# jeong0982/gkr

Measured on AMD Instinct MI355X. Metric: BN254-Fr sumcheck field-ops/sec @ 2^20 vars, higher is better.
Workload: dtype u32x8

## Files before the change

gkr_amd/csrc/capi_internal.h:

```cpp
#pragma once
#include <hip/hip_runtime.h>
#include <sched.h>
#include <stdio.h>
#include <stdlib.h>
#include <string.h>

#include <algorithm>
#include <chrono>
#include <condition_variable>
#include <map>
#include <memory>
#include <mutex>
#include <string>
#include <thread>
#include <vector>

#include "../../include/gkr_amd.h"
#include "fr64.h"
#include "host_cpus.h"
#include "hostpool.h"
#include "kernels.h"
#include "options.h"
#include "gate_seg.h"
#include "keccak.h"
// ... 151 lines not shown
        for (auto p : r) (void)hipFree(p);
        for (auto& g : lists) g.release();
        gt.clear();
        l.clear();
        r.clear();
        lists.clear();
    }
};

struct ProveCrew;

struct AsyncWorker {
    std::thread th;
    std::mutex mu;
    std::condition_variable cv;
    std::function<void()> task;
    bool busy = false, stop = false;
    void loop() {
        std::unique_lock<std::mutex> g(mu);
        for (;;) {
            cv.wait(g, [this] { return stop || (busy && task); });
            if (stop) return;
            std::function<void()> t = std::move(task);
            task = nullptr;
            g.unlock();
            t();
            g.lock();
            busy = false;
            cv.notify_all();
        }
    }
    void run(std::function<void()> fn) {
        std::unique_lock<std::mutex> g(mu);
        if (!th.joinable()) th = std::thread([this] { loop(); });
        cv.wait(g, [this] { return !busy; });
        task = std::move(fn);
        busy = true;
        cv.notify_all();
    }
    void wait() {
        std::unique_lock<std::mutex> g(mu);
        cv.wait(g, [this] { return !busy; });
    }
    ~AsyncWorker() {
        {
            std::unique_lock<std::mutex> g(mu);
            cv.wait(g, [this] { return !busy; });
            stop = true;
            cv.notify_all();
        }
        if (th.joinable()) th.join();
    }
};

struct gkr_ctx {
    int device = 0;
    std::vector<int> devices;
    int host_threads = 0;
    gkr::Options options = gkr::Options::from_environment();
    std::vector<std::unique_ptr<PreparedCircuit>> circuits;
    hipStream_t stream = nullptr;
    hipStream_t aux = nullptr;
    hipStream_t late = nullptr;
    hipStream_t chain = nullptr;
    std::vector<hipEvent_t> aux_events;
    Fr* d_cts = nullptr;
    int transcript = GKR_TRANSCRIPT_HOST;
    std::string err;
    int profile = 0;
    std::map<std::string, ProfileRow> prof;
    std::vector<PendingEvent> pending;
    std::vector<hipEvent_t> event_pool;
    char name[256] = {0};
    uint32_t ticket = 0;
    std::unique_ptr<gkr::SpinPool> pool;
    std::unique_ptr<gkr::SpinPool> solo_pool;
    std::unique_ptr<AsyncWorker> copier;
    std::unique_ptr<AsyncWorker> liner;
    void* mle_arrivals_zeroed = nullptr;
    void* arrivals_zeroed = nullptr;
    void* gate_arrive_zeroed = nullptr;
    bool crew_member = false;
    int help_share = 0;
    int rounds_ahead = 0;
    std::unique_ptr<ProveCrew, void (*)(ProveCrew*)> crew{nullptr, nullptr};
    std::map<std::string, std::pair<void*, size_t>> ws;
    std::map<std::string, std::pair<void*, size_t>> pinned;

    hipError_t workspace(const char* slot, size_t bytes, void** out) {
        auto& e = ws[slot];
        if (e.second < bytes) {
            if (e.first) (void)device_free(e.first);
            e.first = nullptr;
            e.second = 0;
            hipError_t rc = device_malloc(&e.first, bytes);
            if (rc != hipSuccess) return rc;
            e.second = bytes;
        }
        *out = e.first;
        return hipSuccess;
    }
    hipError_t pinned_host(const char* slot, size_t bytes, void** out) {
        auto& e = pinned[slot];
        if (e.second < bytes) {
            if (e.first) (void)hipHostFree(e.first);
            e.first = nullptr;
            e.second = 0;
            hipError_t rc = hipHostMalloc(&e.first, bytes, hipHostMallocCoherent | hipHostMallocMapped);
            if (rc != hipSuccess) return rc;
            memset(e.first, 0, bytes);
            e.second = bytes;
        }
        *out = e.first;
        return hipSuccess;
    }
    void release_buffers() {
        for (auto& c : circuits) c->release();
        circuits.clear();
        for (auto& kv : ws)
            if (kv.second.first) (void)device_free(kv.second.first);
        ws.clear();
        for (auto& kv : pinned)
            if (kv.second.first) (void)hipHostFree(kv.second.first);
        pinned.clear();
    }
    int threads() const { return host_threads > 0 ? host_threads : default_host_threads(); }
    gkr::SpinPool* host_pool() {
        if (crew_member) {
            if (!solo_pool) solo_pool.reset(new gkr::SpinPool(0));
            return solo_pool.get();
        }
        if (!pool) pool.reset(new gkr::SpinPool(threads() - 1));
        return pool.get();
    }
    hipError_t late_stream(hipStream_t* out) {
        if (!late) {
            const hipError_t rc = hipStreamCreateWithFlags(&late, hipStreamNonBlocking);
            if (rc != hipSuccess) return rc;
        }
        *out = late;
        return hipSuccess;
    }
    hipError_t chain_stream(hipStream_t* out) {
        if (!chain) {
            hipError_t rc = hipStreamCreateWithFlags(&chain, hipStreamNonBlocking);
            if (rc != hipSuccess) return rc;
        }
        *out = chain;
        return hipSuccess;
    }
    hipError_t aux_stream(int events) {
        if (!aux) {
            hipError_t rc = hipStreamCreateWithFlags(&aux, hipStreamNonBlocking);
            if (rc != hipSuccess) return rc;
        }
        while ((int)aux_events.size() < events) {
            hipEvent_t e;
            hipError_t rc = hipEventCreateWithFlags(&e, hipEventDisableTiming);
            if (rc != hipSuccess) return rc;
            aux_events.push_back(e);
        }
        return hipSuccess;
    }

    int fail(int status, const std::string& what) {
        err = what;
// ... 77 lines not shown
        }
    }
};

#define GKR_ENTER(ctx)                                        \
    HIP_TRY(ctx, hipSetDevice((ctx)->device));                \
    gkr::OptionScope gkr_option_scope_(&(ctx)->options)

#define HIP_TRY(ctx, expr)                                   \
    do {                                                     \
        hipError_t _e = (expr);                              \
        if (_e != hipSuccess) return (ctx)->hip_fail(_e, #expr); \
    } while (0)


namespace gkr_host {


template <typename T>
struct DevBuf {
    T* p = nullptr;
    ~DevBuf() {
        if (p) (void)hipFree(p);
    }
    hipError_t alloc(size_t count) { return hipMalloc(reinterpret_cast<void**>(&p), count * sizeof(T)); }
};

template <typename Run>
int run_on_upload(gkr_ctx* ctx, const gkr_fr* host, size_t count, Run run) {
    GKR_ENTER(ctx);
    DevBuf<Fr> d;
    HIP_TRY(ctx, d.alloc(count));
    HIP_TRY(ctx, hipMemcpyAsync(d.p, host, count * sizeof(Fr), hipMemcpyHostToDevice, ctx->stream));
    return run(d.p);
}
template <typename Run>
int run_on_tables(gkr_ctx* ctx, const gkr_fr* tables, size_t count, Run run) {
    if (!all_canonical(tables, count)) return ctx->fail(GKR_ERR_NON_CANONICAL, "table entry >= r");
    return run_on_upload(ctx, tables, count, run);
}

struct ThreadTimeAccount {
    double own_pieces_us = 0, helped_us = 0, spin_us = 0;
};
inline thread_local ThreadTimeAccount t_account;
struct HostAccountTotals {
    std::atomic<uint64_t> own_ns{0}, helped_ns{0}, spin_ns{0}, rest_ns{0}, lent_ns{0}, lent_idle_ns{0}, calls{0}, wake_ns{0};
    std::atomic<uint64_t> pieces{0}, piece_ns{0}, piece_pass_ns{0}, lanes[17] = {};
    std::atomic<bool> on{false};
};
inline HostAccountTotals& host_account_totals() {
    static HostAccountTotals t;
    return t;
}
inline bool accounting_on() { return host_account_totals().on.load(std::memory_order_relaxed); }
inline void account_piece(int transcripts, double pass_us, double total_us) {
    HostAccountTotals& t = host_account_totals();
    t.pieces.fetch_add(1, std::memory_order_relaxed);
    t.piece_ns.fetch_add((uint64_t)(total_us * 1e3), std::memory_order_relaxed);
    t.piece_pass_ns.fetch_add((uint64_t)(pass_us * 1e3), std::memory_order_relaxed);
    t.lanes[transcripts < 1 ? 1 : (transcripts > 16 ? 16 : transcripts)].fetch_add(1, std::memory_order_relaxed);
}
inline double now_us_dbg() { return std::chrono::duration<double, std::micro>(std::chrono::steady_clock::now().time_since_epoch()).count(); }

inline bool help_enabled() {
    static const bool on = !gkr::process_switch("GKR_NO_HELP");
    return on;
}
static void run_pieces(gkr::SpinPool* pool, const std::function<bool()>* work, bool several, int priority = 0) {
    auto run = [&] {
        if (pool)
            pool->run_now(work);
        else
            while ((*work)()) {
            }
    };
    const bool dbg = gkr::debug_timing() || accounting_on();
    const double t0 = dbg ? now_us_dbg() : 0.0;
    if (several && help_enabled()) {
        gkr::HelpBoard::Posted posted(work, priority);
        run();
    } else {
        run();
    }
    if (dbg) t_account.own_pieces_us += now_us_dbg() - t0;
}

template <typename Rec>
inline int wait_records(gkr_ctx* ctx, const volatile Rec* recs, int count, uint32_t ticket) {
    const auto t0 = std::chrono::steady_clock::now();
    const bool help = help_enabled();
    auto last_progress = t0;
    for (int b = 0; b < count; ++b) {
        uint32_t spins = 0, helped = 0;
        while (__atomic_load_n(&recs[b].seq, __ATOMIC_ACQUIRE) != ticket) {
            const bool dbg = gkr::debug_timing() || accounting_on();
            const double th0 = dbg ? now_us_dbg() : 0.0;
            const bool did_help = help && gkr::HelpBoard::instance().help();
            if (!did_help) GKR_CPU_RELAX();
            if (dbg) (did_help ? t_account.helped_us : t_account.spin_us) += now_us_dbg() - th0;
            if (did_help ? (++helped & 0x3F) == 0 : (++spins & 0xFFFF) == 0) {
                hipError_t q = hipStreamQuery(ctx->stream);
                if (q != hipSuccess && q != hipErrorNotReady) return ctx->hip_fail(q, "stream failed while waiting for a round");
                if (std::chrono::steady_clock::now() - last_progress > std::chrono::seconds(30)) {
                    if (q == hipSuccess && __atomic_load_n(&recs[b].seq, __ATOMIC_ACQUIRE) == ticket) break;
                    return ctx->fail(GKR_ERR_HIP, "timed out waiting for the device to publish a round");
                }
            }
        }
        if (spins | helped) last_progress = std::chrono::steady_clock::now();
    }
    return GKR_OK;
}

constexpr int kMaxGroups = 32;
constexpr int kMleShardTailLog2 = 6;

#define WS(ctx, slot, type, count, ptr) \
    HIP_TRY(ctx, (ctx)->workspace(slot, (size_t)(count) * sizeof(type), reinterpret_cast<void**>(&(ptr))))

inline int mle_pass_rounds(int m, int n, int jmax) {
    int j = m < jmax ? m : jmax;
    if (((size_t)1 << m) > gkr::kSmallPassEntries && m != n && j > m - 6) j = m - 6;
    if (jmax > 3 && (m - j == 10 || m - j == 11) && m - 12 >= 1) j = m - 12;
    return j < 1 ? 1 : j;
}

constexpr int kMleFirstFoldLevels = 2;
constexpr int kMleTwoLevelRounds = 2 * gkr::kMlePassMaxRounds;
inline bool mle_two_level_first_fold(int n, const gkr::Options& o) {
    const long long levels = o.v[gkr::OPT_first_fold_levels] == 1 || o.v[gkr::OPT_first_fold_levels] == 2 ? o.v[gkr::OPT_first_fold_levels] : kMleFirstFoldLevels;
    return levels == 2 && n >= 18 && n <= 24 && !o.v[gkr::OPT_no_mfma_fold] && o.v[gkr::OPT_rounds_per_pass] <= 0;
}

inline void write_round_output(gkr_fr* out_coeffs, uint32_t* out_len, gkr_fr* out_r, size_t row, const void* c0, const void* c1, uint32_t ln,
                               const void* r) {
    memset(&out_coeffs[row * 2], 0, 32);
    if (ln == 2) memcpy(&out_coeffs[row * 2], c1, 32);
    memcpy(&out_coeffs[row * 2 + 1], c0, 32);
    out_len[row] = ln;
    memcpy(&out_r[row], r, 32);
}
struct GroupHandoff {
    int b0 = 0, nb = 0;
    int state = 0;
    uint32_t ticket = 0;
    std::atomic<uint64_t> claim{0};
    std::atomic<int> done{0};
    template <typename Rec>
    bool records_landed(const Rec* rec) const {
        for (int i = nb - 1; i >= 0; --i)
            if (__atomic_load_n(&rec[b0 + i].seq, __ATOMIC_ACQUIRE) != ticket) return false;
        return true;
    }
    void open(uint32_t generation) {
        done.store(0, std::memory_order_relaxed);
        claim.store((uint64_t)generation << 32, std::memory_order_release);
        state = 1;
    }
    uint32_t open_generation() const {
        const uint64_t c = claim.load(std::memory_order_acquire);
        return (uint32_t)c < (uint32_t)nb ? (uint32_t)(c >> 32) : 0u;
    }
    bool try_claim(uint32_t chunk, uint32_t* first, uint32_t* take, uint32_t* generation = nullptr) {
        uint64_t c = claim.load(std::memory_order_acquire);
        while ((c >> 32) != 0 && (uint32_t)c < (uint32_t)nb) {
// ... 124 lines not shown
```

gkr_amd/csrc/capi_layer.hip:

```cpp
#include "capi_internal.h"

namespace gkr_host {

void host_prod_pass_scalar(const uint64_t* recs, size_t rec_row_words, int count, int J, const uint32_t (*vec_len)[16],
                                  uint64_t (*c2)[16][4], uint64_t (*lin)[16][4], uint64_t (*c0)[16][4], uint64_t (*r)[16][4],
                                  uint64_t* weights, size_t w_row_words) {
    using namespace gkr::h64;
    const F* cts = host_mimc_constants64();
    const F one_m = to_mont(F{{1, 0, 0, 0}});
    for (int k = 0; k < count; ++k) {
        F M[64], SY[8], rm[gkr::kProdMaxJ];
        const F* rec = reinterpret_cast<const F*>(recs + (size_t)k * rec_row_words);
        const int n = 1 << J;
        for (int a = 0; a < n; ++a) {
            for (int b = 0; b < n; ++b) M[a * 8 + b] = rec[a * 8 + b];
            SY[a] = rec[64 + a];
        }
        for (int t = 0; t < J; ++t) {
            const int half = 1 << (J - t - 1);
            F p00 = M[0], p01 = M[half], p10 = M[half * 8], p11 = M[half * 8 + half], s0 = SY[0], s1 = SY[half];
            for (int x = 1; x < half; ++x) {
                p00 = add(p00, M[x * 8 + x]);
                p01 = add(p01, M[x * 8 + half + x]);
                p10 = add(p10, M[(half + x) * 8 + x]);
// ... 201 lines not shown
    return GKR_OK;
}

struct RankExchange {
    gkr_ctx* ctx;
    const LayerShardArgs* shard;
    hipStream_t s;
    uint32_t* h_xflag = nullptr;
    int sums = 0;

    int sum(Fr* d_a, Fr* d_b, size_t each, const uint32_t* d_flag, int local_fail) {
        ++sums;
        if (shard->dev) {
            Timed t(ctx, "exchange", 0.0);
            long long* limbs = reinterpret_cast<long long*>(shard->dev->d_limbs);
            gkr::launch_exchange_widen(d_a, d_b, (uint32_t)each, d_flag, local_fail ? 1u : 0u, limbs, s);
            const int arc = shard->dev->fn(shard->dev->user, (2 * each + 1) * 8, static_cast<void*>(s));
            gkr::launch_exchange_narrow(limbs, d_a, d_b, (uint32_t)each, h_xflag, s);
            if (arc) return ctx->fail(GKR_ERR_INVALID, "the device sum-over-ranks hook failed (status " + std::to_string(arc) + ")");
            HIP_TRY(ctx, hipGetLastError());
            return local_fail;
        }
        const auto t0 = std::chrono::steady_clock::now();
        gkr_fr* buf = nullptr;
        HIP_TRY(ctx, ctx->pinned_host("layer.xbuf", sizeof(gkr_fr) * (2 * each + 1), reinterpret_cast<void**>(&buf)));
        uint32_t hflag = local_fail ? 1u : 0u;
        gkr::launch_copy_words(d_a, buf, each * 8, s);
        gkr::launch_copy_words(d_b, buf + each, each * 8, s);
        if (d_flag && !local_fail && hipMemcpyAsync(&hflag, d_flag, 4, hipMemcpyDeviceToHost, s) != hipSuccess) hflag = 1u;
        const hipError_t se = hipStreamSynchronize(s);
        if (se != hipSuccess) hflag = 1u;
        buf[2 * each] = gkr_fr{{(uint64_t)(hflag != 0), 0, 0, 0}};
        const int arc = shard->allreduce(shard->user, buf, 2 * each + 1);
        if (se != hipSuccess) return ctx->hip_fail(se, "hipStreamSynchronize before the sum over ranks");
        if (arc) return ctx->fail(GKR_ERR_INVALID, "the sum-over-ranks hook failed (status " + std::to_string(arc) + ")");
        if (!all_canonical(buf, 2 * each + 1)) return ctx->fail(GKR_ERR_NON_CANONICAL, "the sum-over-ranks hook returned a value >= r");
        const bool some_failed = (buf[2 * each].l[0] | buf[2 * each].l[1] | buf[2 * each].l[2] | buf[2 * each].l[3]) != 0;
        gkr::launch_copy_words(buf, d_a, each * 8, s);
        gkr::launch_copy_words(buf + each, d_b, each * 8, s);
        if (ctx->profile == 1)
            ctx->add_host_sample("exchange", std::chrono::duration<double, std::milli>(std::chrono::steady_clock::now() - t0).count());
        if (local_fail) return local_fail;
        if (some_failed) return ctx->fail(GKR_ERR_INVALID, "gate type or operand index out of range, or another failure, on some rank");
        return GKR_OK;
    }
    bool flagged() const { return h_xflag && __atomic_load_n(h_xflag, __ATOMIC_ACQUIRE); }
    int check() const { return flagged() ? ctx->fail(GKR_ERR_INVALID, "gate type or operand index out of range, or another failure, on some rank") : GKR_OK; }
};

static int queue_c_phase_setup(LayerRun& R, const LayerPinned& P, RankExchange& xch, uint32_t jp, bool wu_in_host_tail, gkr_fr* const* out_r) {
    const uint32_t k = (uint32_t)R.k, k_i = (uint32_t)R.k_i, batch = (uint32_t)R.batch;
    for (uint32_t b = 0; b < batch; ++b) memcpy(P.u + (size_t)b * k, out_r[b], sizeof(gkr_fr) * k);
    const gkr::CPhaseFuse fuse{wu_in_host_tail ? P.tail : R.Wb, P.pw, R.X, R.Y, jp};
    gkr::launch_eq_table(reinterpret_cast<const Fr*>(P.u), k, 0u, k, R.eq, true, batch, R.s, R.wu ? &fuse : nullptr, R.wu,
                         (uint32_t)(wu_in_host_tail ? 3 * P.tail_stride() : R.wlen));
    bool c_tables_done = false;
    {
        Timed t(R.ctx, "gate_rows", (double)R.span.count * 8.0 * batch);
        if (R.wide) {
            const gkr::WideCFuse wfuse{R.wu, R.X, R.Y};
            gkr::launch_gate_rows_wide(R.span, k_i, k, R.g->plan, R.gate_eq(), R.eq, R.A, R.M, R.lb, R.item_partials, R.gate_arrive, R.s, R.sets, R.plan_counts,
                                       R.wu ? &wfuse : nullptr);
            c_tables_done = R.wu != nullptr;
        } else
            c_tables_done = gkr::launch_gate_rows(R.span, k_i, k, R.g->offsets, R.g->cursor, R.g->list, R.e_hi, R.e_lo, R.kl, R.eq, R.A, R.M, R.lb, &R.g->segs,
                                                  R.seg_partials, R.s, R.shard ? nullptr : &fuse, R.sets);
    }
    if (R.shard)
        if (const int rc = xch.sum(R.A, R.M, R.wlen, nullptr, GKR_OK)) return rc;
    if (!c_tables_done) gkr::launch_prod_c_setup(R.Wb, jp, P.pw, R.A, R.M, R.X, R.Y, k, (uint32_t)R.wlen, batch, R.s);
    return GKR_OK;
}

struct HostPass {
    const LayerPinned* pin;
    int batch, k;
    bool ifma;
    gkr_fr* const* out_coeffs;
    uint32_t* const* out_len;
    gkr_fr* const* out_r;
    uint32_t J, round0, tail_m, tail_jp;
    bool on_host;
    int chunk;
    std::atomic<int> next{0};
};

static bool host_pass_piece(HostPass& hp) {
    const LayerPinned& P = *hp.pin;
    const int first = hp.next.fetch_add(hp.chunk, std::memory_order_relaxed);
    if (first >= hp.batch) return false;
    const int cnt = hp.batch - first < hp.chunk ? hp.batch - first : hp.chunk;
    uint64_t c2[gkr::kProdMaxJ][16][4], lin[gkr::kProdMaxJ][16][4], c0[gkr::kProdMaxJ][16][4], rr[gkr::kProdMaxJ][16][4];
    uint32_t vl[gkr::kProdMaxJ][16];
    const bool acct = accounting_on();
    const double tp0 = acct ? now_us_dbg() : 0.0;
    if (hp.on_host)
        for (int i = 0; i < cnt; ++i)
            host_tail_pass(reinterpret_cast<gkr::h64::F*>(P.tail + (size_t)(first + i) * 3 * P.tail_stride()), P.tail_stride(), hp.tail_m, hp.tail_jp,
                           reinterpret_cast<const gkr::h64::F*>(P.pw + (size_t)(first + i) * 8), hp.J, reinterpret_cast<gkr::h64::F*>(&P.prec[first + i].v[0]));
    for (uint32_t t = 0; t < hp.J; ++t)
        for (int i = 0; i < cnt; ++i) vl[t][i] = 2u + (P.dep[(size_t)(first + i) * 32 + (hp.round0 + t) % hp.k] ? 1u : 0u);
    (hp.ifma && cnt >= 3 ? gkr::gkr_ifma_prod_pass : host_prod_pass_scalar)(
        reinterpret_cast<const uint64_t*>(P.prec + first), sizeof(gkr::ProdPassRec) / 8, cnt, (int)hp.J, vl, c2, lin, c0, rr,
        reinterpret_cast<uint64_t*>(P.pw + (size_t)first * 8), 32);
    const double tp1 = acct ? now_us_dbg() : 0.0;
    for (int i = 0; i < cnt; ++i) {
        const int b = first + i;
        for (uint32_t t = 0; t < hp.J; ++t) {
            const uint32_t round = hp.round0 + t;
            gkr_fr* oc = hp.out_coeffs[b] + (size_t)round * 3;
            memset(&oc[0], 0, 32);
            if (vl[t][i] == 3) memcpy(&oc[0], c2[t][i], 32);
            memcpy(&oc[1], lin[t][i], 32);
            memcpy(&oc[2], c0[t][i], 32);
            hp.out_len[b][round] = vl[t][i];
            memcpy(&hp.out_r[b][round], rr[t][i], 32);
        }
    }
    if (acct) account_piece(cnt, tp1 - tp0, now_us_dbg() - tp0);
    return true;
}

static int run_layer_passes(LayerRun& R, const LayerPinned& P, RankExchange& xch, gkr_fr* const* out_coeffs, uint32_t* const* out_len, gkr_fr* const* out_r) {
    gkr_ctx* ctx = R.ctx;
    const int batch = R.batch, k = R.k;
    Fr* d_ppart = nullptr;
    WS(ctx, "layer.ppart", Fr, (size_t)batch * gkr::prod_pass_scratch_values((uint32_t)k), d_ppart);
    unsigned char* d_fold_plans = nullptr;
    if (k >= 14) WS(ctx, "layer.foldplans", unsigned char, (size_t)batch * gkr::prod_fold_plan_bytes(), d_fold_plans);
    uint32_t* d_arrivals = nullptr;
    if (!gkr::opt(gkr::OPT_no_fused_publish)) {
        WS(ctx, "layer.arrivals", uint32_t, (size_t)(batch < 4096 ? 4096 : batch), d_arrivals);
        if (ctx->arrivals_zeroed != d_arrivals) {
            HIP_TRY(ctx, hipMemsetAsync(d_arrivals, 0, sizeof(uint32_t) * (size_t)(batch < 4096 ? 4096 : batch), R.s));
            ctx->arrivals_zeroed = d_arrivals;
        }
    }
    gkr::SpinPool* pool = batch >= 16 ? ctx->host_pool() : nullptr;
    const bool ifma = host_ifma_ready();
    const bool dbg_sections = gkr::debug_timing();
    double us_launch = 0, us_wait = 0, us_pieces = 0, us_phase1 = 0;
    const double t_passes0 = dbg_sections ? now_us_dbg() : 0.0;
    gkr::SpinPool::Session session(pool, nullptr);
    uint32_t round0 = 0, jp = 0, tail_m = 0;
    bool tail_active = false;
    int rc = GKR_OK;
    for (int phase = 0; phase < 2 && rc == GKR_OK; ++phase) {
        if (phase == 1) {
            const bool wu_in_host_tail = tail_active && R.wu;
            if (tail_active && !wu_in_host_tail) gkr::launch_copy_rows(P.tail, 3 * P.tail_stride() * 8, R.Wb, R.wlen * 8, 8u << jp, (uint32_t)batch, R.s);
            const double t_ph1 = dbg_sections ? now_us_dbg() : 0.0;
            rc = queue_c_phase_setup(R, P, xch, jp, wu_in_host_tail, out_r);
            if (dbg_sections) us_phase1 += now_us_dbg() - t_ph1;
            if (rc) break;
            jp = 0;
            tail_active = false;
        }
        Fr *const Tw = phase ? R.Wc : R.Wb, *const Tx = phase ? R.X : R.U, *const Ty = phase ? R.Y : R.V;
        uint32_t m = (uint32_t)k;
        for (uint32_t rem = (uint32_t)k; rem > 0 && rc == GKR_OK;) {
            const uint32_t J = rem < (uint32_t)gkr::kProdMaxJ ? rem : (uint32_t)gkr::kProdMaxJ;
            const bool on_host = tail_active;
            const bool exports = P.tail && !on_host && m - jp <= P.tail_log2 && rem > J;
            if (!on_host) {
                const uint32_t ticket = ++ctx->ticket;
                const double tl0 = dbg_sections ? now_us_dbg() : 0.0;
                {
                    Timed t(ctx, "layer_prod_pass", 0.0);
                    gkr::launch_prod_pass(Tw, Tx, Ty, m, jp, P.pw, J, d_ppart, (uint32_t)R.wlen, P.prec, ticket, (uint32_t)batch, R.s, d_arrivals, d_fold_plans,
                                          exports ? P.tail : nullptr, (uint32_t)P.tail_stride());
                }
                if (hipError_t le = hipGetLastError(); le != hipSuccess) {
                    rc = ctx->hip_fail(le, "launch of a layer pass");
                    break;
                }
                const double tl1 = dbg_sections ? now_us_dbg() : 0.0;
                rc = wait_records(ctx, P.prec, batch, ticket);
                if (dbg_sections) {
                    us_launch += tl1 - tl0;
                    us_wait += now_us_dbg() - tl1;
                }
                if (!rc) rc = xch.check();
                if (rc) break;
            }
            const int chunk = hash_chunk_size(batch, pool ? pool->workers() + 1 : 1, ctx->crew_member ? ctx->help_share : 0);
            HostPass hp{&P, batch, k, ifma, out_coeffs, out_len, out_r, J, round0, on_host ? tail_m : 0u, jp, on_host, chunk};
            const std::function<bool()> work = [&hp]() -> bool { return host_pass_piece(hp); };
            m -= jp;
            const double tw0 = dbg_sections ? now_us_dbg() : 0.0;
            run_pieces(pool, &work, batch > chunk, ctx->rounds_ahead + (int)(2 * k - round0));
            if (dbg_sections) us_pieces += now_us_dbg() - tw0;
            if (exports) tail_active = true;
            if (exports || on_host) tail_m = m;
            jp = J;
            round0 += J;
            rem -= J;
        }
    }
    session.close();
    if (dbg_sections)
        fprintf(stderr, "[gkr timing] layer k_i=%d k=%d batch=%d passes: %.0f us = launch calls %.0f + waiting for records %.0f + hashing pieces %.0f + c-phase set-up calls %.0f + other %.0f\n",
                R.k_i, k, batch, now_us_dbg() - t_passes0, us_launch, us_wait, us_pieces, us_phase1,
                now_us_dbg() - t_passes0 - us_launch - us_wait - us_pieces - us_phase1);
    return rc;
}

static int run_layer_gates(gkr_ctx* ctx, int batch, int k_i, int k, const uint8_t* d_gt, const uint32_t* d_l, const uint32_t* d_r, const gkr_fr* z,
                           const Fr* d_W, gkr_fr* const* out_coeffs, uint32_t* const* out_len, gkr_fr* const* out_r, const LayerShardArgs* shard,
                           GateLists* cached, const LayerGroup* group) {
    hipStream_t s = ctx->stream;
    const bool lists_fresh = !(cached && cached->ready);
    LayerRun R{ctx, s, batch, k_i, k, (size_t)1 << k, gkr::GateSpan{shard ? shard->gate_base : 0, shard ? shard->gate_count : (uint64_t)1 << k_i}};
    LayerPinned P;
    R.wide = layer_is_wide(R.span, k_i, k);
    R.kl = gkr::gate_seg_shift(R.span, (uint32_t)k_i, (uint32_t)k);
    R.shard = shard;
    R.sets = group ? group->d_sets : nullptr;
    R.plan_counts = group ? &group->plan_counts : (lists_fresh ? nullptr : &cached->plan_counts);
    R.lb = gkr::LayerBatch{(uint32_t)batch, 0u, R.wlen, R.wlen};
    R.g = cached ? cached : &R.ws_lists;
    if (!lists_fresh && R.wide && !R.g->plan) return ctx->fail(GKR_ERR_INVALID, "cached gate lists were built without the wide layer's item plan");
    if (const int rc = alloc_layer_run(R, P)) return rc;
    memcpy(P.z, z, sizeof(gkr_fr) * (size_t)batch * k_i);
    const bool dep_wide = k > 13;
    uint32_t* dep_bits = nullptr;
    if (dep_wide) WS(ctx, "layer.depbits", uint32_t, (size_t)batch, dep_bits);
    gkr::launch_layer_prologue(reinterpret_cast<const Fr*>(P.z), (uint32_t)k_i, (uint32_t)k_i - R.kl, R.kl, R.e_hi, R.e_lo, d_W, R.Wb, R.Wc, (uint32_t)k,
                               dep_wide ? nullptr : R.dep, P.dep, (uint32_t)batch, s, dep_bits);
    if (dep_wide) gkr::launch_depends_wide(d_W, (uint32_t)k, dep_bits, R.dep, P.dep, (uint32_t)batch, s, true);
    if (R.wide) {
        const size_t words = gkr::gate_plan_arrive_words(R.span.count, (uint32_t)k) * (size_t)batch;
        const size_t alloc = words < 4096 ? 4096 : words;
        WS(ctx, "gates.arrive", uint32_t, alloc, R.gate_arrive);
        if (ctx->gate_arrive_zeroed != R.gate_arrive || words > 4096) {
            HIP_TRY(ctx, hipMemsetAsync(R.gate_arrive, 0, alloc * sizeof(uint32_t), s));
            ctx->gate_arrive_zeroed = R.gate_arrive;
        }
        if (R.E) {
            Timed t(ctx, "eq_table_z", ((double)batch * 32.0) * (double)((size_t)1 << k_i));
            gkr::launch_eq_outer(R.e_hi, R.e_lo, (uint32_t)k_i, R.kl, R.E, (uint32_t)batch, s);
        }
    }
    if (lists_fresh) {
        if (const int rc = queue_gate_lists(ctx, R.span, k_i, k, d_gt, d_l, d_r, R.wide, R.g, cached != nullptr, &R.bad)) return rc;
        if (cached) cached->ready = true;
    }
    {
        Timed t(ctx, "gate_uv", (double)R.span.count * 8.0 * batch);
        if (R.wide)
            gkr::launch_gate_uv_wide(R.span, (uint32_t)k_i, (uint32_t)k, R.g->plan, R.gate_eq(), R.Wc, R.U, R.V, R.lb, R.item_partials, R.gate_arrive, s, R.sets, R.plan_counts);
        else
            gkr::launch_gate_uv(R.span, (uint32_t)k_i, (uint32_t)k, R.g->offsets, R.g->cursor, R.g->list, R.e_hi, R.e_lo, R.kl, R.Wc, R.U, R.V, R.lb, &R.g->segs, R.seg_partials, s, R.sets);
    }
    RankExchange xch{ctx, shard, s};
    if (shard && shard->dev) {
        HIP_TRY(ctx, ctx->pinned_host("layer.xflag", 64, reinterpret_cast<void**>(&xch.h_xflag)));
        *xch.h_xflag = 0;
    }
    if (shard)
        if (const int rc = xch.sum(R.U, R.V, R.wlen, lists_fresh ? R.bad : nullptr, GKR_OK)) return rc;
    if (lists_fresh && !(shard && shard->dev))
        if (const int rc = validate_gate_lists(ctx, R.span, k, R.wide, R.bad, R.g, cached != nullptr)) return rc;
    int rc = run_layer_passes(R, P, xch, out_coeffs, out_len, out_r);
    if (rc && shard && xch.sums == 1 && !xch.flagged()) (void)xch.sum(R.A, R.M, R.wlen, nullptr, rc);
    if (rc) {
        (void)hipStreamSynchronize(s);
        ctx->arrivals_zeroed = nullptr;
        return rc;
    }
    HIP_TRY(ctx, hipGetLastError());
    HIP_TRY(ctx, hipStreamSynchronize(s));
    if ((rc = xch.check())) return rc;
    ctx->drain_events();
// ... 322 lines not shown
```

gkr_amd/csrc/capi_prove.hip:

```cpp
#include "capi_internal.h"

namespace gkr_host {

void mobius_msb(std::vector<gkr::h64::F>& c, int k) {
    const size_t n = (size_t)1 << k;
    for (int b = 0; b < k; ++b) {
        const size_t bit = (size_t)1 << (k - 1 - b);
        for (size_t i = 0; i < n; ++i)
            if (i & bit) c[i] = gkr::h64::sub(c[i], c[i ^ bit]);
    }
}

void line_restriction(const std::vector<gkr::h64::F>& vals, const std::vector<gkr::h64::F>& coeffs, int k, const gkr_fr* b,
                      const gkr_fr* c, gkr_fr* out, uint32_t* out_len) {
    using gkr::h64::F;
    const F zero = {{0, 0, 0, 0}};
    int maxdeg = 0;
    const size_t n = (size_t)1 << k;
    for (size_t mono = 0; mono < n; ++mono)
        if (!gkr::h64::is_zero(coeffs[mono])) {
            const int deg = __builtin_popcountll((unsigned long long)mono);
            if (deg > maxdeg) maxdeg = deg;
        }
    const size_t stride = (size_t)k + 1;
// ... 141 lines not shown
        uint64_t w;
        memcpy(&w, q + i, 8);
        h1 = (h1 ^ w) * 0x100000001b3ULL;
        h2 = (h2 + w) * 0xBF58476D1CE4E5B9ULL;
        h2 ^= h2 >> 29;
    }
    for (; i < n; ++i) {
        h1 = (h1 ^ q[i]) * 0x100000001b3ULL;
        h2 = (h2 + q[i]) * 0x94D049BB133111EBULL;
    }
    *out_h1 = h1;
    *out_h2 = h2;
}
static void fold_segment_hashes(uint32_t depth, const uint64_t* seg_hashes, size_t n_segments, uint64_t* out_h1, uint64_t* out_h2) {
    uint64_t h1 = 0xcbf29ce484222325ULL ^ depth, h2 = 0x9E3779B97F4A7C15ULL + n_segments;
    for (size_t i = 0; i < n_segments; ++i) {
        h1 = (h1 ^ seg_hashes[2 * i]) * 0x100000001b3ULL;
        h2 = (h2 + seg_hashes[2 * i + 1]) * 0xBF58476D1CE4E5B9ULL;
        h2 ^= h2 >> 29;
    }
    *out_h1 = h1;
    *out_h2 = h2;
}

static int find_or_upload_circuit(gkr_ctx* ctx, const gkr_circuit_desc* c, uint64_t h1, uint64_t h2, PreparedCircuit** out,
                                  std::unique_ptr<PreparedCircuit>& fresh) {
    const uint32_t L = c->depth;
    hipStream_t s = ctx->stream;
    *out = nullptr;
    for (size_t i = 0; i < ctx->circuits.size(); ++i)
        if (ctx->circuits[i]->h1 == h1 && ctx->circuits[i]->h2 == h2 && ctx->circuits[i]->k.size() == L + 1 &&
            memcmp(ctx->circuits[i]->k.data(), c->k, (L + 1) * sizeof(uint32_t)) == 0 && retained_gate_bytes_match(c, ctx->circuits[i]->retained)) {
            std::unique_ptr<PreparedCircuit> hit = std::move(ctx->circuits[i]);
            ctx->circuits.erase(ctx->circuits.begin() + i);
            ctx->circuits.push_back(std::move(hit));
            *out = ctx->circuits.back().get();
            return GKR_OK;
        }
    for (uint32_t i = 0; i < L; ++i) {
        const size_t gates = (size_t)1 << c->k[i];
        for (size_t g = 0; g < gates; ++g)
            if (c->gate_type[i][g] > 1 || (c->left[i][g] >> c->k[i + 1]) || (c->right[i][g] >> c->k[i + 1]))
                return ctx->fail(GKR_ERR_INVALID, "gate type or operand index out of range");
    }
    fresh.reset(new PreparedCircuit());
    fresh->h1 = h1;
    fresh->h2 = h2;
    fresh->k.assign(c->k, c->k + L + 1);
    fresh->lists.resize(L);
    retain_gate_bytes(c, fresh->retained);
    for (uint32_t i = 0; i < L; ++i) {
        const size_t gates = (size_t)1 << c->k[i];
        uint8_t* dg = nullptr;
        uint32_t *dl_ = nullptr, *dr_ = nullptr;
        HIP_TRY(ctx, hipMalloc(reinterpret_cast<void**>(&dg), gates));
        fresh->gt.push_back(dg);
        HIP_TRY(ctx, hipMalloc(reinterpret_cast<void**>(&dl_), gates * 4));
        fresh->l.push_back(dl_);
        HIP_TRY(ctx, hipMalloc(reinterpret_cast<void**>(&dr_), gates * 4));
        fresh->r.push_back(dr_);
        HIP_TRY(ctx, hipMemcpyAsync(dg, c->gate_type[i], gates, hipMemcpyHostToDevice, s));
        HIP_TRY(ctx, hipMemcpyAsync(dl_, c->left[i], gates * 4, hipMemcpyHostToDevice, s));
        HIP_TRY(ctx, hipMemcpyAsync(dr_, c->right[i], gates * 4, hipMemcpyHostToDevice, s));
    }
    HIP_TRY(ctx, hipStreamSynchronize(s));
    *out = fresh.get();
    return GKR_OK;
}

static bool k_list_groupable(const uint32_t* k, uint32_t depth) {
    for (uint32_t i = 0; i < depth; ++i) {
        const gkr::GateSpan span{0, (uint64_t)1 << k[i]};
        if (gkr::gate_segs_words(span, k[i], k[i + 1]) != 0) return false;
    }
    return true;
}

static int prove_group_impl(gkr_ctx* ctx, const gkr_prove_item* members, int n_members) {
    using gkr::h64::F;
    const auto t_entry = std::chrono::steady_clock::now();
    if (!members || n_members < 1) return ctx->fail(GKR_ERR_INVALID, "no members");
    GKR_ENTER(ctx);
    const gkr_circuit_desc* c = members[0].circuit;
    int rc = GKR_OK;
    int batch = 0;
    for (int m = 0; m < n_members; ++m) {
        const gkr_prove_item& it = members[m];
        rc = check_circuit(ctx, it.circuit);
        if (rc) return rc;
        if (!it.input_values || !it.outs || it.batch < 1 || it.batch > 4096) return ctx->fail(GKR_ERR_INVALID, "null pointer or batch out of [1, 4096]");
        if (it.circuit->depth != c->depth || memcmp(it.circuit->k, c->k, (c->depth + 1) * sizeof(uint32_t)) != 0)
            return ctx->fail(GKR_ERR_INVALID, "the circuits of a lockstep group must share their k list");
        batch += it.batch;
    }
    if (batch > 4096) return ctx->fail(GKR_ERR_INVALID, "more than 4096 proofs in one group");
    std::vector<gkr_proof_buf> outs_v((size_t)batch);
    std::vector<int> member_of((size_t)batch), first_of((size_t)n_members);
    {
        int b = 0;
        for (int m = 0; m < n_members; ++m) {
            first_of[m] = b;
            for (int i = 0; i < members[m].batch; ++i, ++b) {
                outs_v[b] = members[m].outs[i];
                member_of[b] = m;
            }
        }
    }
    gkr_proof_buf* const outs = outs_v.data();
    for (int b = 0; b < batch; ++b) {
        const gkr_proof_buf* out = &outs[b];
        if (!out->sumcheck_coeffs || !out->sumcheck_len || !out->sumcheck_r || !out->q || !out->q_len || !out->z || !out->r ||
            !out->d_coeffs || !out->input_coeffs)
            return ctx->fail(GKR_ERR_INVALID, "null pointer in proof buffers");
    }
    const uint32_t L = c->depth;
    for (int m = 0; m < n_members; ++m)
        for (uint32_t i = 0; i < L; ++i)
            if (!members[m].circuit->gate_type[i] || !members[m].circuit->left[i] || !members[m].circuit->right[i])
                return ctx->fail(GKR_ERR_INVALID, "null gate array");
    if (n_members > 1 && (ctx->transcript != GKR_TRANSCRIPT_HOST || !k_list_groupable(c->k, L)))
        return ctx->fail(GKR_ERR_INVALID, "a lockstep group needs the host transcript and layers below the segment form's size");
    const size_t n_in = (size_t)1 << c->k[L];
    const bool dbg_pre = gkr::debug_timing();
    auto us_since_entry = [&] { return std::chrono::duration<double, std::micro>(std::chrono::steady_clock::now() - t_entry).count(); };
    const bool check_on_device = n_in * (size_t)batch >= ((size_t)1 << 16);
    if (!check_on_device)
        for (int m = 0; m < n_members; ++m)
            if (!all_canonical(members[m].input_values, n_in * members[m].batch)) return ctx->fail(GKR_ERR_NON_CANONICAL, "input value >= r");
    const double us_canon = us_since_entry();
    hipStream_t s = ctx->stream;

    const bool no_cache = gkr::opt(gkr::OPT_no_circuit_cache) != 0;
    std::vector<PreparedCircuit*> pcs((size_t)n_members, nullptr);
    std::vector<std::unique_ptr<PreparedCircuit>> fresh((size_t)n_members);
    struct DropFresh {
        gkr_ctx* ctx;
        std::vector<std::unique_ptr<PreparedCircuit>>& v;
        ~DropFresh() {
            bool any = false;
            for (auto& p : v) any |= (bool)p;
            if (any) (void)hipStreamSynchronize(ctx->stream);
            for (auto& p : v)
                if (p) p->release();
        }
    } drop_fresh{ctx, fresh};
    std::vector<uint64_t> hs((size_t)2 * n_members);
    {
        std::vector<HashSegment> segs;
        std::vector<size_t> first_seg((size_t)n_members + 1, 0);
        size_t total_bytes = 0;
        for (int m = 0; m < n_members; ++m) {
            circuit_hash_segments(members[m].circuit, segs);
            first_seg[(size_t)m + 1] = segs.size();
        }
        for (const HashSegment& sg : segs) total_bytes += sg.n;
        std::vector<uint64_t> seg_hashes(2 * segs.size());
        std::atomic<size_t> next{0};
        const std::function<bool()> work = [&]() -> bool {
            const size_t i = next.fetch_add(1, std::memory_order_relaxed);
            if (i >= segs.size()) return false;
            const size_t m = (size_t)(std::upper_bound(first_seg.begin(), first_seg.end(), i) - first_seg.begin()) - 1;
            hash_segment(segs[i], i - first_seg[m], &seg_hashes[2 * i], &seg_hashes[2 * i + 1]);
            return true;
        };
        gkr::SpinPool* hash_pool = (!ctx->crew_member && total_bytes >= ((size_t)2 << 20)) ? ctx->host_pool() : nullptr;
        gkr::SpinPool::Session session(hash_pool, nullptr);
// ... 215 lines not shown
    } liner;
    for (uint32_t i = 0; i < L; ++i) {
        const int k_i = c->k[i], k = c->k[i + 1];
        for (int b = 0; b < batch; ++b) {
            scp[b] = outs[b].sumcheck_coeffs + row_off * 3;
            slp[b] = outs[b].sumcheck_len + row_off;
            srp[b] = outs[b].sumcheck_r + row_off;
        }
        const bool line_prepared = i + 1 == L && k > 12 && ctx->profile == 0;
        if (line_prepared) {
            if (!ctx->liner) ctx->liner.reset(new AsyncWorker());
            liner.worker = ctx->liner.get();
            liner.started = true;
            const int device = ctx->device;
            const Fr* Wn = dW[i + 1];
            const uint32_t ub = (uint32_t)batch, uk = (uint32_t)k;
            hipStream_t aux = ctx->aux;
            const gkr::Options* const call_options = &ctx->options;
            ctx->liner->run([=]() {
                gkr::OptionScope option_scope(call_options);
                if (hipSetDevice(device) != hipSuccess) return;
                gkr::launch_line_restriction(Wn, uk, nullptr, d_lr, d_lrdeg, nullptr, nullptr, nullptr, ub, aux, gkr::LinePart::prepare);
            });
        }
        const auto tl0 = std::chrono::steady_clock::now();
        ctx->rounds_ahead = 0;
        for (uint32_t later = i + 1; later < L; ++later) ctx->rounds_ahead += 2 * (int)c->k[later + 1];
        rc = run_layer_batch(ctx, batch, k_i, k, pc->gt[i], pc->l[i], pc->r[i], z_cur.data(), dW[i + 1], scp.data(), slp.data(),
                             srp.data(), nullptr, &pc->lists[i], n_members > 1 ? &groups[i] : nullptr);
        ctx->rounds_ahead = 0;
        if (rc) {
            liner.finish();
            (void)hipStreamSynchronize(ctx->aux);
            return rc;
        }
        const auto tl1 = std::chrono::steady_clock::now();
        std::vector<gkr_fr> z_next((size_t)batch * k);
        {
            gkr_fr* lines = h_lines + (size_t)i * batch * 2 * kmax;
            for (int b = 0; b < batch; ++b) memcpy(lines + (size_t)b * 2 * k, srp[b], (size_t)2 * k * sizeof(gkr_fr));
            const Fr* Wn = dW[i + 1];
            Fr* bcm = d_lrbc + (size_t)i * batch * 2 * kmax;
            Fr* qdst = d_q + q_off * batch;
            uint32_t* qlen_dst = d_qlen + (size_t)i * batch;
            hipStream_t aux = ctx->aux;
            if (k > 12 && ctx->profile == 0) {
                if (!ctx->liner) ctx->liner.reset(new AsyncWorker());
                liner.worker = ctx->liner.get();
                liner.started = true;
                const int device = ctx->device;
                const uint32_t ub = (uint32_t)batch, uk = (uint32_t)k;
                const gkr::Options* const call_options = &ctx->options;
                ctx->liner->run([=]() {
                    gkr::OptionScope option_scope(call_options);
                    if (hipSetDevice(device) != hipSuccess) return;
                    gkr::launch_line_restriction(Wn, uk, reinterpret_cast<const Fr*>(lines), d_lr, d_lrdeg, bcm, qdst, qlen_dst, ub, aux,
                                                 line_prepared ? gkr::LinePart::finish : gkr::LinePart::all);
                });
            } else {
                Timed t(ctx, "line_restriction", 0.0, ctx->aux, true);
                gkr::launch_line_restriction(Wn, (uint32_t)k, reinterpret_cast<const Fr*>(lines), d_lr, d_lrdeg, bcm, qdst, qlen_dst, (uint32_t)batch, aux);
            }
        }
        auto finish = [&](int b) {
            const gkr_fr* sr = srp[b];
            const gkr_fr* b_star = sr;
            const gkr_fr* c_star = sr + k;
            const gkr_fr r_star = sr[2 * k - 1];
            outs[b].r[i] = r_star;
            F rs;
            memcpy(&rs, &r_star, 32);
            rs = gkr::h64::to_mont(rs);
            gkr_fr* zn = outs[b].z + z_off + k_i;
            for (int j = 0; j < k; ++j) {
                F bj, cj;
                memcpy(&bj, &b_star[j], 32);
                memcpy(&cj, &c_star[j], 32);
                const F v = gkr::h64::add(bj, gkr::h64::mont_mul(gkr::h64::sub(cj, bj), rs));
                memcpy(&zn[j], &v, 32);
                memcpy(&z_next[(size_t)b * k + j], &v, 32);
            }
        };
        {
            std::atomic<int> next{0};
            const std::function<bool()> work = [&]() -> bool {
                const int b = next.fetch_add(1, std::memory_order_relaxed);
                if (b >= batch) return false;
                finish(b);
                return true;
            };
            gkr::SpinPool::Session session(pool, nullptr);
            run_pieces(pool, &work, batch > 1);
        }
        if (dbg_pb)
            fprintf(stderr, "[gkr timing] prove layer %u: sumcheck %.0f us, q / z on the host %.0f us (since entry of the hand-off: %.0f us)\n", i,
                    std::chrono::duration<double, std::micro>(tl1 - tl0).count(),
                    std::chrono::duration<double, std::micro>(std::chrono::steady_clock::now() - tl1).count(),
                    std::chrono::duration<double, std::micro>(std::chrono::steady_clock::now() - tpb0).count());
        z_cur.swap(z_next);
        row_off += (size_t)2 * k;
        q_off += (size_t)k + 1;
        z_off += (size_t)k_i;
    }
    {
        HIP_TRY(ctx, hipGetLastError());
        copier.finish();
        liner.finish();
        HIP_TRY(ctx, hipStreamSynchronize(ctx->aux));
        if (h_in_flag) return ctx->fail(GKR_ERR_NON_CANONICAL, "input value >= r");
        for (int b = 0; b < batch; ++b) {
            if (members[member_of[b]].require_zero_output && !gkr::h64::is_zero(hW0_first ? hW0_first[b] : hW[0][(size_t)b << c->k[0]]))
                return ctx->fail(GKR_ERR_INVALID, "output 0 is not zero (convert.rs:838 asserts d_values[0] == 0)");
            std::vector<F> co;
            if (!coeffs_done[0]) {
                co.assign(hW[0] + ((size_t)b << c->k[0]), hW[0] + ((size_t)(b + 1) << c->k[0]));
                mobius_msb(co, c->k[0]);
                memcpy(outs[b].d_coeffs, co.data(), co.size() * sizeof(F));
            }
            if (!coeffs_done[1]) {
                co.assign(hW[1] + ((size_t)b << c->k[L]), hW[1] + ((size_t)(b + 1) << c->k[L]));
                mobius_msb(co, c->k[L]);
                memcpy(outs[b].input_coeffs, co.data(), co.size() * sizeof(F));
            }
        }

        const F* hq = reinterpret_cast<const F*>(d_q);
        const uint32_t* hqlen = d_qlen;
        size_t off = 0;
        for (uint32_t i = 0; i < L; ++i) {
            const size_t kq = (size_t)c->k[i + 1] + 1;
            for (int b = 0; b < batch; ++b) {
                memcpy(outs[b].q + off, &hq[off * batch + (size_t)b * kq], kq * sizeof(F));
                outs[b].q_len[i] = hqlen[(size_t)i * batch + b];
            }
            off += kq;
        }
    }
    if (dbg_pb) {
        const auto us = [](auto a, auto b) { return std::chrono::duration<double, std::micro>(b - a).count(); };
        const auto t_end = std::chrono::steady_clock::now();
        fprintf(stderr, "[gkr timing] prove batch=%d depth=%u: %.0f us before the layers (circuit lookup, forward evaluation, readback), "
                        "%.0f us layers + q readback, since entry %.0f us\n", batch, L, us(t_entry, tpb0), us(tpb0, t_end), us(t_entry, t_end));
        fprintf(stderr, "[gkr timing] this thread: own hashing pieces (incl. waiting for helpers) %.0f us, others' pieces %.0f us, spinning with nothing to take %.0f us, "
                        "the rest (launches, set-up, copies) %.0f us\n", t_account.own_pieces_us, t_account.helped_us, t_account.spin_us,
                us(t_entry, t_end) - t_account.own_pieces_us - t_account.helped_us - t_account.spin_us);
    }
    if (account) {
        HostAccountTotals& tot = host_account_totals();
        const double all_us = std::chrono::duration<double, std::micro>(std::chrono::steady_clock::now() - t_entry).count();
        const double rest = all_us - t_account.own_pieces_us - t_account.helped_us - t_account.spin_us;
        tot.own_ns.fetch_add((uint64_t)(t_account.own_pieces_us * 1e3), std::memory_order_relaxed);
        tot.helped_ns.fetch_add((uint64_t)(t_account.helped_us * 1e3), std::memory_order_relaxed);
        tot.spin_ns.fetch_add((uint64_t)(t_account.spin_us * 1e3), std::memory_order_relaxed);
        tot.rest_ns.fetch_add((uint64_t)((rest > 0 ? rest : 0) * 1e3), std::memory_order_relaxed);
        tot.calls.fetch_add(1, std::memory_order_relaxed);
    }
    copier.finish();
    if (copier.err != hipSuccess) return ctx->hip_fail(copier.err, "copy of the d / input_func coefficients to the proof buffers");
    for (auto& f : fresh) {
        if (!f || no_cache) continue;
        constexpr size_t kMaxCachedCircuits = 64;
        if (ctx->circuits.size() >= kMaxCachedCircuits) {
            ctx->circuits.front()->release();
            ctx->circuits.erase(ctx->circuits.begin());
        }
        ctx->circuits.push_back(std::move(f));
    }
    return GKR_OK;
}

static int prove_batch_impl(gkr_ctx* ctx, const gkr_circuit_desc* c, const gkr_fr* input_values, int batch, int require_zero_output,
                            gkr_proof_buf* outs) {
    gkr_prove_item one{c, input_values, batch, require_zero_output, outs, 0};
    return prove_group_impl(ctx, &one, 1);
}
// ... 252 lines not shown
```

gkr_amd/csrc/hostpool.h:

```cpp
#pragma once
#include <atomic>
#include <condition_variable>
#include <functional>
#include <mutex>
#include <thread>
#include <vector>

#if defined(__x86_64__)
#include <immintrin.h>
#define GKR_CPU_RELAX() _mm_pause()
#else
#define GKR_CPU_RELAX() ((void)0)
#endif

namespace gkr {

class HelpBoard {
   public:
    static HelpBoard& instance() {
        static HelpBoard board;
        return board;
    }
    int post(const std::function<bool()>* work, int priority = 0) {
        for (int i = 0; i < kSlots; ++i) {
            const std::function<bool()>* expected = nullptr;
            if (slots_[i].job.compare_exchange_strong(expected, work, std::memory_order_seq_cst)) {
                slots_[i].priority.store(priority, std::memory_order_relaxed);
                posted_.fetch_add(1, std::memory_order_seq_cst);
                return i;
            }
        }
        return -1;
    }
    void retire(int slot) {
        if (slot < 0) return;
        slots_[slot].job.store(nullptr, std::memory_order_seq_cst);
        posted_.fetch_sub(1, std::memory_order_seq_cst);
        while (slots_[slot].inside.load(std::memory_order_seq_cst) != 0) GKR_CPU_RELAX();
    }
    bool help() {
        if (posted_.load(std::memory_order_acquire) == 0) return false;
        const int start = next_.fetch_add(1, std::memory_order_relaxed);
        uint64_t tried = 0;
        for (;;) {
            int best = -1, best_prio = 0;
            for (int n = 0; n < kSlots; ++n) {
                const int i = (start + n) % kSlots;
                if ((tried >> i) & 1u) continue;
                if (slots_[i].job.load(std::memory_order_acquire) == nullptr) continue;
                const int pr = slots_[i].priority.load(std::memory_order_relaxed);
                if (best < 0 || pr > best_prio) {
                    best = i;
                    best_prio = pr;
                }
            }
            if (best < 0) return false;
            tried |= (uint64_t)1 << best;
            Slot& sl = slots_[best];
            sl.inside.fetch_add(1, std::memory_order_seq_cst);
            const std::function<bool()>* job = sl.job.load(std::memory_order_seq_cst);
            const bool did = job && (*job)();
            sl.inside.fetch_sub(1, std::memory_order_seq_cst);
            if (did) return true;
        }
    }

    class Posted {
       public:
        explicit Posted(const std::function<bool()>* work, int priority = 0) : slot_(HelpBoard::instance().post(work, priority)) {}
        ~Posted() { HelpBoard::instance().retire(slot_); }
        Posted(const Posted&) = delete;
        Posted& operator=(const Posted&) = delete;

       private:
        int slot_;
    };

   private:
    static constexpr int kSlots = 64;
    struct alignas(64) Slot {
        std::atomic<const std::function<bool()>*> job{nullptr};
        std::atomic<int> inside{0};
        std::atomic<int> priority{0};
    };
    Slot slots_[kSlots];
    std::atomic<int> posted_{0};
    std::atomic<unsigned> next_{0};
};

class SpinPool {
   public:
    explicit SpinPool(int workers) {
        for (int i = 0; i < workers; ++i) threads_.emplace_back([this] { worker(); });
    }
    ~SpinPool() {
        {
            std::lock_guard<std::mutex> g(mu_);
            stop_.store(true);
        }
        cv_.notify_all();
        for (auto& t : threads_) t.join();
    }
    int workers() const { return (int)threads_.size(); }

    void begin_session(const std::function<bool()>* try_work) {
        {
            std::lock_guard<std::mutex> g(mu_);
            fn_ = try_work;
            session_.fetch_add(1, std::memory_order_release);
        }
        cv_.notify_all();
    }
    void run_now(const std::function<bool()>* work) {
        job_.store(work, std::memory_order_seq_cst);
        while ((*work)()) {
        }
        job_.store(nullptr, std::memory_order_seq_cst);
        while (job_busy_.load(std::memory_order_seq_cst) != 0) GKR_CPU_RELAX();
    }

    void end_session() {
        session_.fetch_add(1, std::memory_order_seq_cst);
        while (inside_.load(std::memory_order_seq_cst) != 0) GKR_CPU_RELAX();
    }

    class Session {
       public:
        Session(SpinPool* pool, const std::function<bool()>* try_work) : pool_(pool) {
            if (pool_) pool_->begin_session(try_work);
        }
        ~Session() { close(); }
        Session(const Session&) = delete;
        Session& operator=(const Session&) = delete;
        void close() {
            if (pool_) pool_->end_session();
            pool_ = nullptr;
        }

       private:
        SpinPool* pool_;
    };

   private:
    void worker() {
        for (;;) {
            uint64_t s = session_.load(std::memory_order_acquire);
            if (!(s & 1)) {
                std::unique_lock<std::mutex> g(mu_);
                cv_.wait(g, [this] { return stop_.load() || (session_.load() & 1); });
                if (stop_.load()) return;
                continue;
            }
            inside_.fetch_add(1, std::memory_order_seq_cst);
            if (session_.load(std::memory_order_seq_cst) == s) {
                const std::function<bool()>* fn = fn_;
                unsigned idle = 0;
                while (session_.load(std::memory_order_acquire) == s) {
                    bool did = false;
                    if (fn) {
                        did = (*fn)();
                    } else {
                        job_busy_.fetch_add(1, std::memory_order_seq_cst);
                        const std::function<bool()>* job = job_.load(std::memory_order_seq_cst);
                        if (job) did = (*job)();
                        job_busy_.fetch_sub(1, std::memory_order_seq_cst);
                    }
                    if (!did) did = HelpBoard::instance().help();
                    if (did) {
// ... 26 lines not shown
```

Measured before the change: 500.3 billion.

## Replace posted std::function work-sharing with indexed help-board units

Adds a fixed table of work units to the HelpBoard, where each unit holds a generation-tagged countdown that helpers claim by CAS, then run an indexed function pointer. The host product pass and the per-batch finish loop now submit indexed pieces through these units instead of a std::function lambda with a shared atomic counter. Each prove call holds one persistent unit. The aim is to cut posting and unposting overhead and let idle threads pick the highest-priority unit. The cost is added concurrency complexity, such as generation reuse and helpers scanning units.

Result: no change. 500.7 billion (median of 2 runs) (+0.1%).

```diff
diff --git a/gkr_amd/csrc/capi_internal.h b/gkr_amd/csrc/capi_internal.h
--- a/gkr_amd/csrc/capi_internal.h
+++ b/gkr_amd/csrc/capi_internal.h
@@ -257,6 +257,7 @@
     void* gate_arrive_zeroed = nullptr;
     bool crew_member = false;
     int help_share = 0;
+    gkr::HelpBoard::Unit* help_unit = nullptr;
     int rounds_ahead = 0;
     std::unique_ptr<ProveCrew, void (*)(ProveCrew*)> crew{nullptr, nullptr};
     std::map<std::string, std::pair<void*, size_t>> ws;
@@ -500,6 +501,30 @@
         run();
     } else {
         run();
+    }
+    if (dbg) t_account.own_pieces_us += now_us_dbg() - t0;
+}
+
+static void run_unit_pieces(gkr_ctx* ctx, gkr::SpinPool* pool, void (*fn)(void*, int), void* arg, int pieces, int priority) {
+    const bool dbg = gkr::debug_timing() || accounting_on();
+    const double t0 = dbg ? now_us_dbg() : 0.0;
+    auto run = [&](gkr::HelpBoard::Unit& unit) {
+        if (pool && pool->workers() > 0) {
+            const std::function<bool()> take = [&unit]() -> bool { return unit.take_one(); };
+            unit.open(fn, arg, pieces, priority);
+            pool->run_now(&take);
+            unit.finish();
+        } else {
+            unit.run(fn, arg, pieces, priority);
+        }
+    };
+    if (pieces == 1) {
+        fn(arg, 0);
+    } else if (ctx->help_unit) {
+        run(*ctx->help_unit);
+    } else {
+        gkr::HelpBoard::Unit unit(help_enabled());
+        run(unit);
     }
     if (dbg) t_account.own_pieces_us += now_us_dbg() - t0;
 }
diff --git a/gkr_amd/csrc/capi_layer.hip b/gkr_amd/csrc/capi_layer.hip
--- a/gkr_amd/csrc/capi_layer.hip
+++ b/gkr_amd/csrc/capi_layer.hip
@@ -307,13 +307,12 @@
     uint32_t J, round0, tail_m, tail_jp;
     bool on_host;
     int chunk;
-    std::atomic<int> next{0};
 };
 
-static bool host_pass_piece(HostPass& hp) {
+static void host_pass_piece(void* arg, int index) {
+    HostPass& hp = *static_cast<HostPass*>(arg);
     const LayerPinned& P = *hp.pin;
-    const int first = hp.next.fetch_add(hp.chunk, std::memory_order_relaxed);
-    if (first >= hp.batch) return false;
+    const int first = index * hp.chunk;
     const int cnt = hp.batch - first < hp.chunk ? hp.batch - first : hp.chunk;
     uint64_t c2[gkr::kProdMaxJ][16][4], lin[gkr::kProdMaxJ][16][4], c0[gkr::kProdMaxJ][16][4], rr[gkr::kProdMaxJ][16][4];
     uint32_t vl[gkr::kProdMaxJ][16];
@@ -343,7 +342,6 @@
         }
     }
     if (acct) account_piece(cnt, tp1 - tp0, now_us_dbg() - tp0);
-    return true;
 }
 
 static int run_layer_passes(LayerRun& R, const LayerPinned& P, RankExchange& xch, gkr_fr* const* out_coeffs, uint32_t* const* out_len, gkr_fr* const* out_r) {
@@ -410,10 +408,9 @@
             }
             const int chunk = hash_chunk_size(batch, pool ? pool->workers() + 1 : 1, ctx->crew_member ? ctx->help_share : 0);
             HostPass hp{&P, batch, k, ifma, out_coeffs, out_len, out_r, J, round0, on_host ? tail_m : 0u, jp, on_host, chunk};
-            const std::function<bool()> work = [&hp]() -> bool { return host_pass_piece(hp); };
             m -= jp;
             const double tw0 = dbg_sections ? now_us_dbg() : 0.0;
-            run_pieces(pool, &work, batch > chunk, ctx->rounds_ahead + (int)(2 * k - round0));
+            run_unit_pieces(ctx, pool, host_pass_piece, &hp, (batch + chunk - 1) / chunk, ctx->rounds_ahead + (int)(2 * k - round0));
             if (dbg_sections) us_pieces += now_us_dbg() - tw0;
             if (exports) tail_active = true;
             if (exports || on_host) tail_m = m;
diff --git a/gkr_amd/csrc/capi_prove.hip b/gkr_amd/csrc/capi_prove.hip
--- a/gkr_amd/csrc/capi_prove.hip
+++ b/gkr_amd/csrc/capi_prove.hip
@@ -247,6 +247,12 @@
     if (!members || n_members < 1) return ctx->fail(GKR_ERR_INVALID, "no members");
     GKR_ENTER(ctx);
     const gkr_circuit_desc* c = members[0].circuit;
+    gkr::HelpBoard::Unit help_unit(help_enabled());
+    struct HelpUnitScope {
+        gkr_ctx* ctx;
+        ~HelpUnitScope() { ctx->help_unit = nullptr; }
+    } help_unit_scope{ctx};
+    ctx->help_unit = &help_unit;
     int rc = GKR_OK;
     int batch = 0;
     for (int m = 0; m < n_members; ++m) {
@@ -628,15 +634,8 @@
             }
         };
         {
-            std::atomic<int> next{0};
-            const std::function<bool()> work = [&]() -> bool {
-                const int b = next.fetch_add(1, std::memory_order_relaxed);
-                if (b >= batch) return false;
-                finish(b);
-                return true;
-            };
             gkr::SpinPool::Session session(pool, nullptr);
-            run_pieces(pool, &work, batch > 1);
+            run_unit_pieces(ctx, pool, [](void* f, int b) { (*static_cast<decltype(finish)*>(f))(b); }, &finish, batch, 0);
         }
         if (dbg_pb)
             fprintf(stderr, "[gkr timing] prove layer %u: sumcheck %.0f us, q / z on the host %.0f us (since entry of the hand-off: %.0f us)\n", i,
diff --git a/gkr_amd/csrc/hostpool.h b/gkr_amd/csrc/hostpool.h
--- a/gkr_amd/csrc/hostpool.h
+++ b/gkr_amd/csrc/hostpool.h
@@ -38,7 +38,115 @@
         posted_.fetch_sub(1, std::memory_order_seq_cst);
         while (slots_[slot].inside.load(std::memory_order_seq_cst) != 0) GKR_CPU_RELAX();
     }
+    struct alignas(64) UnitEntry {
+        std::atomic<uint64_t> state{0};
+        std::atomic<int> done{0};
+        std::atomic<int> priority{0};
+        std::atomic<int> owned{0};
+        void (*fn)(void*, int) = nullptr;
+        void* arg = nullptr;
+        int total = 0;
+        int claim() {
+            uint64_t s = state.load(std::memory_order_acquire);
+            while ((uint32_t)s != 0) {
+                if (state.compare_exchange_weak(s, s - 1, std::memory_order_acquire, std::memory_order_acquire)) return total - (int)(uint32_t)s;
+            }
+            return -1;
+        }
+        void run_claimed(int index) {
+            fn(arg, index);
+            done.fetch_add(1, std::memory_order_release);
+        }
+    };
+    class Unit {
+       public:
+        explicit Unit(bool shared = true) : e_(&own_) {
+            if (shared) {
+                HelpBoard& b = instance();
+                for (int i = 0; i < kUnits; ++i) {
+                    int expected = 0;
+                    if (b.units_[i].owned.load(std::memory_order_relaxed) == 0 &&
+                        b.units_[i].owned.compare_exchange_strong(expected, 1, std::memory_order_acquire)) {
+                        e_ = &b.units_[i];
+                        int hi = b.units_hi_.load(std::memory_order_relaxed);
+                        while (hi < i + 1 && !b.units_hi_.compare_exchange_weak(hi, i + 1, std::memory_order_relaxed)) {
+                        }
+                        break;
+                    }
+                }
+            }
+        }
+        ~Unit() {
+            if (e_ != &own_) e_->owned.store(0, std::memory_order_release);
+        }
+        Unit(const Unit&) = delete;
+        Unit& operator=(const Unit&) = delete;
+        bool on_board() const { return e_ != &own_; }
+
+        void open(void (*fn)(void*, int), void* arg, int pieces, int priority) {
+            e_->fn = fn;
+            e_->arg = arg;
+            e_->total = pieces;
+            e_->done.store(0, std::memory_order_relaxed);
+            e_->priority.store(priority, std::memory_order_relaxed);
+            const uint64_t gen = (e_->state.load(std::memory_order_relaxed) >> 32) + 1;
+            e_->state.store(gen << 32 | (uint32_t)pieces, std::memory_order_release);
+        }
+        bool take_one() {
+            const int i = e_->claim();
+            if (i < 0) return false;
+            e_->run_claimed(i);
+            return true;
+        }
+        void finish() {
+            while (e_->done.load(std::memory_order_acquire) != e_->total) GKR_CPU_RELAX();
+        }
+        void run(void (*fn)(void*, int), void* arg, int pieces, int priority) {
+            if (pieces <= 0) return;
+            open(fn, arg, pieces, priority);
+            while (take_one()) {
+            }
+            finish();
+        }
+
+       private:
+        UnitEntry own_;
+        UnitEntry* e_;
+    };
+
     bool help() {
+        if (help_units()) return true;
+        return help_posted();
+    }
+
+   private:
+    bool help_units() {
+        const int hi = units_hi_.load(std::memory_order_relaxed);
+        if (hi == 0) return false;
+        static thread_local unsigned rotate = 0;
+        const unsigned start = rotate++;
+        for (int attempt = 0; attempt < 4; ++attempt) {
+            UnitEntry* best = nullptr;
+            int best_prio = 0;
+            for (int n = 0; n < hi; ++n) {
+                UnitEntry& u = units_[(start + (unsigned)n) % (unsigned)hi];
+                if ((uint32_t)u.state.load(std::memory_order_relaxed) == 0) continue;
+                const int pr = u.priority.load(std::memory_order_relaxed);
+                if (!best || pr > best_prio) {
+                    best = &u;
+                    best_prio = pr;
+                }
+            }
+            if (!best) return false;
+            const int i = best->claim();
+            if (i >= 0) {
+                best->run_claimed(i);
+                return true;
+            }
+        }
+        return false;
+    }
+    bool help_posted() {
         if (posted_.load(std::memory_order_acquire) == 0) return false;
         const int start = next_.fetch_add(1, std::memory_order_relaxed);
         uint64_t tried = 0;
@@ -65,6 +173,7 @@
         }
     }
 
+   public:
     class Posted {
        public:
         explicit Posted(const std::function<bool()>* work, int priority = 0) : slot_(HelpBoard::instance().post(work, priority)) {}
@@ -84,6 +193,9 @@
         std::atomic<int> priority{0};
     };
     Slot slots_[kSlots];
+    static constexpr int kUnits = 64;
+    UnitEntry units_[kUnits];
+    std::atomic<int> units_hi_{0};
     std::atomic<int> posted_{0};
     std::atomic<unsigned> next_{0};
 };
```
